# MaxChen228/pingpong-selfplay-ai

Hardware: AMD Instinct MI355X
Metric: env-steps/sec (whole node) at 65536 arenas, 1/2/4/8 GPUs; CPU-ref baseline (higher is better)
Workload: dtype f64 env state / f32 QNet; 1 GPU; configs[2]: 65536 arenas/GPU, full DQN train_iterative loop (act both players + env tick + PER push/sample + double-DQN update + Adam + target sync); arenas_per_gpu=65536, global_arenas=65536, pool=8, batch=256, updates_per_vector_step=1, memory_size=1000000, parallelism=dp1 (arena shards, 1 all-reduce/update)

## Files before the change

### pingpong-selfplay-ai_amd/csrc/pm_mfma.h

```cpp
#pragma once
#include "pm_dev.h"

namespace pm {

typedef float f32x16 __attribute__((ext_vector_type(16)));
typedef __attribute__((address_space(3))) void lds_void;

constexpr int PLAIN = 4936;
enum : int {
    F_W1 = 0,
    F_W2 = 512,
    F_B1 = 4608,
    F_B2 = 4672,
    F_H = 4736,
    F_BH = 4992,
    F_SIZE = 5008,
};
static_assert(PLAIN + F_SIZE == PM_QNET_NW, "effective weight block size");

__device__ __forceinline__ int rho(int r) { return (r & 3) + 8 * (r >> 2); }

__device__ __forceinline__ float relu(float x) { return __int_as_float(max(__float_as_int(x), 0)); }

__device__ __forceinline__ void write_feature_frags(const float* __restrict__ p, float* __restrict__ w) {
// ... 242 lines not shown
    for (int t = 0; t < 2; ++t)
#pragma unroll
        for (int r = 0; r < 16; ++r) c1[t][r] = relu(c1[t][r]);
    {
        const float4* b = reinterpret_cast<const float4*>(lw + F_B2 + (jt * 2 + h) * 16);
#pragma unroll
        for (int q4 = 0; q4 < 4; ++q4) {
            const float4 v = b[q4];
            c2[4 * q4 + 0] = v.x; c2[4 * q4 + 1] = v.y; c2[4 * q4 + 2] = v.z; c2[4 * q4 + 3] = v.w;
        }
    }
    const float4* w2 = reinterpret_cast<const float4*>(lw + F_W2) + lane + jt * 8 * 64;
    float4 wcur = w2[0];
#pragma unroll
    for (int g = 0; g < 8; ++g) {
        const int t = g >> 2, rq = g & 3;
        const float4 wnext = w2[((g + 1) & 7) * 64];
        c2 = __builtin_amdgcn_mfma_f32_32x32x2f32(wcur.x, c1[t][4 * rq + 0], c2, 0, 0, 0);
        c2 = __builtin_amdgcn_mfma_f32_32x32x2f32(wcur.y, c1[t][4 * rq + 1], c2, 0, 0, 0);
        c2 = __builtin_amdgcn_mfma_f32_32x32x2f32(wcur.z, c1[t][4 * rq + 2], c2, 0, 0, 0);
        c2 = __builtin_amdgcn_mfma_f32_32x32x2f32(wcur.w, c1[t][4 * rq + 3], c2, 0, 0, 0);
        wcur = wnext;
        __builtin_amdgcn_sched_barrier(0);
    }
}

__device__ __forceinline__ void heads_half(const float* hf, const f32x16& c2, int lane, int t, float (&acc)[4]) {
    const float4* hw = reinterpret_cast<const float4*>(hf + (lane >> 5) * 128) + t * 16;
#pragma unroll
    for (int r = 0; r < 16; ++r) {
        const float x = relu(c2[r]);
        const float4 w = hw[r];
        acc[0] = fmaf(w.x, x, acc[0]);
        acc[1] = fmaf(w.y, x, acc[1]);
        acc[2] = fmaf(w.z, x, acc[2]);
        acc[3] = fmaf(w.w, x, acc[3]);
    }
}

__device__ __forceinline__ void heads_finish(const float (&acc)[4], const float* hf, float (&q)[3]) {
    float v = acc[0], a0 = acc[1], a1 = acc[2], a2 = acc[3];
    v += __shfl_xor(v, 32);
    a0 += __shfl_xor(a0, 32);
    a1 += __shfl_xor(a1, 32);
    a2 += __shfl_xor(a2, 32);
    v += hf[256];
    a0 += hf[257];
    a1 += hf[258];
    a2 += hf[259];
    const float mean = ((a0 + a1) + a2) / 3.0f;
    q[0] = v + (a0 - mean);
    q[1] = v + (a1 - mean);
    q[2] = v + (a2 - mean);
}

__device__ __forceinline__ void tile_inputs(const float* __restrict__ o, int h, float (&xs)[4]) {
    xs[0] = h ? o[0] : 1.0f;
    xs[1] = o[1 + h];
    xs[2] = o[3 + h];
    xs[3] = o[5 + h];
}

struct TilePre {
    bool have;
    float xs[4];
};

__device__ __forceinline__ void run_tiles(const float* lw, const float* __restrict__ obs, const int* list, int count,
                                          const TileOut& out, const TilePre pre) {
    const int lane = threadIdx.x & 63, wave = threadIdx.x >> 6, nw = blockDim.x >> 6;
    const int h = lane >> 5, col = lane & 31;
    const int ntiles = (count + 31) >> 5;
    int tl = wave;
    if (tl >= ntiles) return;
    int arena = list[min(tl * 32 + col, count - 1)];
    float xs[4];
    if (pre.have) {
#pragma unroll
        for (int k = 0; k < 4; ++k) xs[k] = pre.xs[k];
    } else {
        tile_inputs(obs + (size_t)arena * 7, h, xs);
    }
    for (; tl < ntiles; tl += nw) {
        const int row = tl * 32 + col;
        const bool valid = row < count;
        const int tn = tl + nw;
        int arena_n = arena;
        float xn[4] = {xs[0], xs[1], xs[2], xs[3]};
        if (tn < ntiles) {
            arena_n = list[min(tn * 32 + col, count - 1)];
            tile_inputs(obs + (size_t)arena_n * 7, h, xn);
        }
        f32x16 c2[2];
#ifdef PM_DIAG
        if (tl == wave) {
            __builtin_amdgcn_s_waitcnt(0);
            PM_BLK(5);
        }
#endif
        tile_hidden(lw, xs, lane, c2);
#ifdef PM_DIAG
        if (tl == wave) PM_BLK(6);
#endif
        float q[3];
        tile_heads(lw + F_H, c2, lane, q);
#ifdef PM_DIAG
// ... 164 lines not shown
```

### pingpong-selfplay-ai_amd/csrc/pm_rollout.hip

```cpp
#include "pm_host.h"
#include "pm_mfma.h"
#include "pm_per.h"

using namespace pm;

namespace {

constexpr int kRollBlock = 256;
constexpr int kHeadsBlock = 256;
static_assert(PM_ROLL_HEADS == 264, "heads workspace stride: 256 fragment floats + 4 biases + 4 pad");

__global__ __launch_bounds__(kHeadsBlock) void k_rollout_heads(const float* __restrict__ paramsB, uint64_t seed_net,
                                                               uint64_t counter0, float* __restrict__ ws) {
    __shared__ float noise[132];
    __shared__ float heads[260];
    gen_noise(seed_net, TAG_NOISE_ACT, counter0 + blockIdx.x, noise, threadIdx.x, blockDim.x);
    __syncthreads();
    fold_heads_from(paramsB + PM_QNET_HEAD_OFF, nullptr, noise, PM_FOLD_TRAIN_FRESH, heads, nullptr, threadIdx.x,
                    blockDim.x);
    __syncthreads();
    float* hf = ws + (size_t)blockIdx.x * PM_ROLL_HEADS;
    heads_to_frags(heads, hf);
    if (threadIdx.x < 4) hf[260 + threadIdx.x] = 0.f;
}
// ... 176 lines not shown
            if (lane < 32)
#pragma unroll
                for (int k = 0; k < 7; ++k) { sm.ob[0][col][k] = oA[k]; sm.ob[1][col][k] = nB2[k]; }
        } else if (st + 1 < steps) {
            roll_draws(p, sm, i, ctr + 1, (st + 1) & 1, eps, seed_env, wv, lane);
        }
        __syncthreads();
    }
    if (wv == 3 && lane < 32 && valid) {
        store_arena(s, i, a);
        float oA[7], oB[7];
        observe(a, oA, oB);
        store_row7(obsA + (size_t)i * 7, oA);
        store_row7(obsB + (size_t)i * 7, oB);
        rp.ep_reward[i] = er;
    }
    if (!stats) return;
    const bool mine = wv == 3 && lane < 32 && valid;
    long long v[6] = {mine ? fin : 0, mine ? winB : 0, mine ? ptA : 0, mine ? ptB : 0, mine ? winE : 0,
                      mine ? rsum : 0};
#pragma unroll
    for (int k = 0; k < 6; ++k) v[k] = wave_sum(v[k]);
    long long mv = v[0];
#pragma unroll
    for (int k = 1; k < 6; ++k) mv = lane == k ? v[k] : mv;
    if (wv == 3 && lane < 6) atomicAdd(reinterpret_cast<unsigned long long*>(stats + lane), (unsigned long long)mv);
}

__global__ __launch_bounds__(kRollBlock) __attribute__((amdgpu_waves_per_eu(3, 3))) void k_rollout_push(
    const pm_env_params p, const pm_env_state s, const float* __restrict__ wA, const float* __restrict__ wB,
    const float* __restrict__ ws, double eps, uint64_t seed_env, uint64_t counter0, int steps,
    float* __restrict__ obsA, float* __restrict__ obsB, long long* __restrict__ stats, int n, const RollPush rp) {
    rollout_push_body(p, s, wA, wB, ws, eps, seed_env, counter0, steps, obsA, obsB, stats, n, rp);
}

constexpr int kR16Block = 512;

#ifdef PM_DIAG
static __device__ unsigned long long pm_diag_roll[2][8];
#define ROLL_T(k)                                                                 \
    do {                                                                          \
        if (diag) {                                                               \
            const unsigned long long now_ = __builtin_amdgcn_s_memtime();         \
            dacc[(k)] += now_ - dprev;                                            \
            dprev = now_;                                                         \
        }                                                                         \
    } while (0)
#else
#define ROLL_T(k) \
    do {          \
    } while (0)
#endif

__device__ __forceinline__ int l2_pos(int u) {
    const int t = u >> 5, v = u & 31, b = (v >> 2) & 1, r = (v & 3) + 4 * (v >> 3);
    return 2 * (16 * t + r) + b;
}
__device__ __forceinline__ int l2_unit(int q) {
    const int i = q >> 1, b = q & 1;
    return 32 * (i >> 4) + rho(i & 15) + 4 * b;
}
__device__ __forceinline__ int head_pos(int u) {
    const int t = u >> 5, v = u & 31;
    return 16 * t + (v & 3) + 4 * (v >> 3);
}

typedef float f32x4v16 __attribute__((ext_vector_type(4)));

struct Roll16Shared {
    __attribute__((aligned(16))) float img2[2][4][4][64][4];
    __attribute__((aligned(16))) float img1[2][4][64][2];
    __attribute__((aligned(16))) float b2v[2][4][4][4];
    __attribute__((aligned(16))) float hfA[264];
    __attribute__((aligned(16))) float hfB[2][320];
    __attribute__((aligned(16))) float h1s[2][4][4][16][4];
    __attribute__((aligned(16))) float c2s[2][2][8][16][4];
    float ob[2][16][8];
    ServeDraw sdraw[2][16];
    int epsa[2][16];
    __attribute__((aligned(16))) float opw[3][2][4][32];
};

__device__ __forceinline__ void roll16_opw(Roll16Shared& sm, int set, const float* hf) {
    const int lane = threadIdx.x & 63;
#pragma unroll
    for (int it = 0; it < 4; ++it) {
        const int idx = it * 64 + lane, h = idx >> 7, j = (idx >> 5) & 3, q = idx & 31;
        sm.opw[set][h][j][q] = hf[(h * 32 + q) * 4 + j];
    }
}

__device__ __forceinline__ float xor16_sum(float v) {
    const auto r = __builtin_amdgcn_permlane16_swap(__float_as_uint(v), __float_as_uint(v), false, false);
    return __uint_as_float(r[0]) + __uint_as_float(r[1]);
}
__device__ __forceinline__ void halves_bcast(int v, int& lo, int& hi) {
    const auto r = __builtin_amdgcn_permlane32_swap((unsigned)v, (unsigned)v, false, false);
    lo = (int)r[0];
    hi = (int)r[1];
}

__device__ __forceinline__ void roll16_serve(const pm_env_params& p, Roll16Shared& sm, int i, uint64_t ctr, int b,
                                             uint64_t seed, int g) {
    const U4 r = philox((uint32_t)i, g == 1 ? (TAG_SERVE_STEP | 0x100u) : TAG_SERVE_STEP, (uint32_t)ctr,
                        (uint32_t)(ctr >> 32), seed);
    const auto sx = __builtin_amdgcn_permlane16_swap(r.x, r.x, false, false);
    const auto sy = __builtin_amdgcn_permlane16_swap(r.y, r.y, false, false);
    const auto sz = __builtin_amdgcn_permlane16_swap(r.z, r.z, false, false);
    const auto sw = __builtin_amdgcn_permlane16_swap(r.w, r.w, false, false);
    const ServeDraw d = serve_from_blocks(p, r, U4{sx[1], sy[1], sz[1], sw[1]});
    if (g == 0) sm.sdraw[b][threadIdx.x & 15] = d;
}
__device__ __forceinline__ void roll16_eps(Roll16Shared& sm, int i, uint64_t ctr, int b, double eps, uint64_t seed,
                                           int g) {
    if (g == 0) {
        const U4 rr = philox64((uint32_t)i, TAG_ACT, ctr, seed);
        sm.epsa[b][threadIdx.x & 15] = u53(rr.x, rr.y) < eps ? (int)below(rr.z, 3u) : -1;
    }
}

__device__ __forceinline__ void rollout16_body(const pm_env_params& p, const pm_env_state& s, const float* __restrict__ wA,
                                               const float* __restrict__ wB, const float* __restrict__ ws, double eps,
                                               uint64_t seed_env, uint64_t counter0, int steps, float* __restrict__ obsA,
                                               float* __restrict__ obsB, long long* __restrict__ stats, int n) {
    __shared__ Roll16Shared sm;
    const int t = threadIdx.x, lane = t & 63, col = lane & 15, g = lane >> 4;
    const int wv = __builtin_amdgcn_readfirstlane(t >> 6);
    const int player = wv >> 2, rt = wv & 3;
    const int i = blockIdx.x * 16 + col;
    const bool valid = i < n;
    for (int k = t; k < 2 * 4 * 4 * 64 * 4; k += kR16Block) {
        const int pp = k >> 12, r2 = (k >> 10) & 3, s4 = (k >> 8) & 3, ln = (k >> 2) & 63, e = k & 3;
        const float* w = pp ? wB : wA;
        (&sm.img2[0][0][0][0][0])[k] = w[W2 + (16 * r2 + (ln & 15)) * 64 + l2_unit(4 * (4 * s4 + e) + (ln >> 4))];
    }
    for (int k = t; k < 2 * 4 * 64 * 2; k += kR16Block) {
        const int pp = k >> 9, r2 = (k >> 7) & 3, ln = (k >> 1) & 63, sx = k & 1;
        const float* w = pp ? wB : wA;
        const int row = 16 * r2 + (ln & 15), kk = 4 * sx + (ln >> 4);
        (&sm.img1[0][0][0][0])[k] = kk == 0 ? w[B1 + row] : w[W1 + row * 7 + kk - 1];
    }
    if (t < 128) {
        const int pp = t >> 6, r2 = (t >> 4) & 3, gg = (t >> 2) & 3, r = t & 3;
        (&sm.b2v[0][0][0][0])[t] = (pp ? wB : wA)[B2 + 16 * r2 + 4 * gg + r];
    }
    if (t < 260) sm.hfA[t] = t < 256 ? wA[PLAIN + F_H + t] : wA[PLAIN + F_BH + t - 256];
    if (wv == 7) fetch_heads(ws, 0, sm.hfB[0], lane);
    if (wv == 1) roll16_serve(p, sm, i, counter0, 0, seed_env, g);
    if (wv == 2) roll16_eps(sm, i, counter0, 0, eps, seed_env, g);
    Arena a{};
    int fin = 0, winB = 0, ptA = 0, ptB = 0;
    if (wv == 0) {
        a = load_arena(s, valid ? i : n - 1);
        float oA[7], oB[7];
        observe(a, oA, oB);
        if (g < 2)
#pragma unroll
            for (int k = 0; k < 7; ++k) sm.ob[g][col][k] = g ? oB[k] : oA[k];
    }
    asm volatile("s_waitcnt vmcnt(0)" ::: "memory");
    if (wv == 7) roll16_opw(sm, 1, sm.hfB[0]);
    if (wv == 6) roll16_opw(sm, 0, wA + PLAIN + F_H);
    __syncthreads();
    const float4* im2 = reinterpret_cast<const float4*>(sm.img2[player][rt][0][lane]);
    float4 w2r[4];
    const float2 w1r = *reinterpret_cast<const float2*>(sm.img1[player][rt][lane]);
#pragma unroll
    for (int s4 = 0; s4 < 4; ++s4) {
        const float4 w = im2[s4 * 64];
        w2r[s4] = w;
    }
    const float4 b2r = *reinterpret_cast<const float4*>(sm.b2v[player][rt][g]);
#ifdef PM_DIAG
    const bool diag = blockIdx.x == 0 && wv < 2;
    unsigned long long dacc[8] = {0, 0, 0, 0, 0, 0, 0, 0}, dprev = __builtin_amdgcn_s_memtime();
#endif
    for (int st = 0; st < steps; ++st) {
        const uint64_t ctr = counter0 + (uint64_t)st;
        if (wv == 7 && st + 1 < steps) fetch_heads_async(ws, st + 1, sm.hfB[(st + 1) & 1], lane);
        float hw4[32];
        if (wv == 0) {
            const float* src = sm.opw[(lane >> 5) ? 1 + (st & 1) : 0][(lane >> 4) & 1][lane & 3];
#pragma unroll
            for (int k = 0; k < 8; ++k) {
                const float4 w = *reinterpret_cast<const float4*>(src + 4 * k);
                hw4[4 * k] = w.x; hw4[4 * k + 1] = w.y; hw4[4 * k + 2] = w.z; hw4[4 * k + 3] = w.w;
            }
        }
        {
            const float* o = sm.ob[player][col];
            const float o0 = o[g == 0 ? 0 : g - 1];
            const float x0 = g == 0 ? 1.0f : o0, x1 = o[3 + g];
            const f32x4v16 zero = {0.f, 0.f, 0.f, 0.f};
            f32x4v16 c1 = __builtin_amdgcn_mfma_f32_16x16x4f32(w1r.x, x0, zero, 0, 0, 0);
            c1 = __builtin_amdgcn_mfma_f32_16x16x4f32(w1r.y, x1, c1, 0, 0, 0);
#pragma unroll
            for (int r = 0; r < 4; ++r) {
                const int q = l2_pos(16 * rt + 4 * g + r), sq = q >> 2;
                sm.h1s[player][q & 3][sq >> 2][col][sq & 3] = relu(c1[r]);
            }
        }
        ROLL_T(0);
        __syncthreads();
        ROLL_T(1);
        float bs[16];
        {
#pragma unroll
            for (int k = 0; k < 4; ++k) {
                const float4 v = *reinterpret_cast<const float4*>(sm.h1s[player][g][k][col]);
                bs[4 * k] = v.x; bs[4 * k + 1] = v.y; bs[4 * k + 2] = v.z; bs[4 * k + 3] = v.w;
            }
        }
        f32x4v16 c2 = {b2r.x, b2r.y, b2r.z, b2r.w};

#pragma unroll
// ... 13 lines not shown
        if (wv == 7) asm volatile("s_waitcnt vmcnt(0)" ::: "memory");
        ROLL_T(2);
        __syncthreads();
        ROLL_T(3);
        if (wv == 0) {
            const int hp = lane >> 5, hh = (lane >> 4) & 1;
            const float* hf = hp ? sm.hfB[st & 1] : sm.hfA;
            float xb[32];
#pragma unroll
            for (int k = 0; k < 8; ++k) {
                const float4 x = *reinterpret_cast<const float4*>(sm.c2s[hp][hh][k][col]);
                xb[4 * k] = x.x; xb[4 * k + 1] = x.y; xb[4 * k + 2] = x.z; xb[4 * k + 3] = x.w;
            }
            const int ea = sm.epsa[st & 1][col];
            ServeDraw sd = sm.sdraw[st & 1][col];
            f32x4v16 acc = {0.f, 0.f, 0.f, 0.f};
#pragma unroll
            for (int q = 0; q < 32; ++q) acc = __builtin_amdgcn_mfma_f32_4x4x1f32(hw4[q], xb[q], acc, 0, 0, 0);
            __builtin_amdgcn_sched_group_barrier(0x100, 9, 0);
            __builtin_amdgcn_sched_group_barrier(0x008, 32, 0);
            float v = xor16_sum(acc[0]), a0 = xor16_sum(acc[1]), a1 = xor16_sum(acc[2]), a2 = xor16_sum(acc[3]);
            v += hf[256];
            a0 += hf[257];
            a1 += hf[258];
            a2 += hf[259];
            const float mean = ((a0 + a1) + a2) / 3.0f;
            const float qv[3] = {v + (a0 - mean), v + (a1 - mean), v + (a2 - mean)};
            int act = argmax3(qv);
            if (hp) act = ea >= 0 ? ea : act;
            int aA, aB;
            halves_bcast(act, aA, aB);
            ROLL_T(4);
            float rA, rB;
            const int d = tick(p, a, aA, aB, rA, rB);
            ptA += rA > 0.f ? 1 : 0;
            ptB += rB > 0.f ? 1 : 0;
            if (d) {
                fin += 1;
                winB += rB > 0.f ? 1 : 0;
                serve_finish(sd);
                serve(a, sd.vx, sd.vy, sd.spin);
            }
            float oA[7], oB[7];
            observe(a, oA, oB);
            if (g < 2)
#pragma unroll
                for (int k = 0; k < 7; ++k) sm.ob[g][col][k] = g ? oB[k] : oA[k];
            ROLL_T(5);
        } else if (wv == 1 && st + 1 < steps) {
            roll16_serve(p, sm, i, ctr + 1, (st + 1) & 1, seed_env, g);
        } else if (wv == 2 && st + 1 < steps) {
            roll16_eps(sm, i, ctr + 1, (st + 1) & 1, eps, seed_env, g);
        } else if (wv == 7 && st + 1 < steps) {
            roll16_opw(sm, 1 + ((st + 1) & 1), sm.hfB[(st + 1) & 1]);
        }
        __syncthreads();
        ROLL_T(6);
    }
#ifdef PM_DIAG
    if (diag && lane == 0)
#pragma unroll
        for (int k = 0; k < 8; ++k) pm_diag_roll[wv][k] = k < 7 ? dacc[k] : (unsigned long long)steps;
#endif
    if (wv == 0 && g == 0 && valid) {
        store_arena(s, i, a);
        float oA[7], oB[7];
        observe(a, oA, oB);
        store_row7(obsA + (size_t)i * 7, oA);
        store_row7(obsB + (size_t)i * 7, oB);
    }
    if (!stats || wv != 0) return;
    const bool mine = g == 0 && valid;
    long long v[4] = {mine ? fin : 0, mine ? winB : 0, mine ? ptA : 0, mine ? ptB : 0};
#pragma unroll
    for (int k = 0; k < 4; ++k) v[k] = wave_sum(v[k]);
    long long mv = v[0];
#pragma unroll
    for (int k = 1; k < 4; ++k) mv = lane == k ? v[k] : mv;
    if (lane < 4) atomicAdd(reinterpret_cast<unsigned long long*>(stats + lane), (unsigned long long)mv);
}

__global__ __launch_bounds__(kR16Block) void k_rollout16(const pm_env_params p, const pm_env_state s,
                                                         const float* __restrict__ wA, const float* __restrict__ wB,
                                                         const float* __restrict__ ws, double eps, uint64_t seed_env,
                                                         uint64_t counter0, int steps, float* __restrict__ obsA,
                                                         float* __restrict__ obsB, long long* __restrict__ stats,
                                                         int n) {
    rollout16_body(p, s, wA, wB, ws, eps, seed_env, counter0, steps, obsA, obsB, stats, n);
}

}

static int rollout_launch(const pm_env_params* p, const pm_env_state* s, const float* wA, const float* wB,
                          const float* paramsB, float epsilon, uint64_t seed_env, uint64_t seed_net, uint64_t counter0,
                          int32_t steps, float* heads_ws, float* obsA, float* obsB, const RollPush* rp, void* per_work,
                          int64_t* stats, int32_t n, void* stream) {
    const char* name = rp ? "pm_rollout_push" : "pm_rollout";
    PM_REQUIRE(n >= 0 && steps >= 0, PM_E_SIZE, "%s: n=%d steps=%d", name, n, steps);
    if (n == 0 || steps == 0) return PM_OK;
    PM_REQUIRE(p && s && s->x && s->y && s->vx && s->vy && s->spin && s->top && s->bot && s->scoreA && s->scoreB &&
                   s->bounces && wA && wB && paramsB && heads_ws && obsA && obsB,
               PM_E_ARG, "%s: null buffer", name);
    PM_REQUIRE((((uintptr_t)wA) | ((uintptr_t)wB) | ((uintptr_t)heads_ws)) % 16 == 0, PM_E_ARG,
               "%s: wA, wB and heads_ws must be 16-byte aligned", name);
    PM_REQUIRE(p->speed_scale_every > 0, PM_E_ARG, "%s: speed_scale_every must be > 0", name);
    hipStream_t st = pm_stream(stream);
    hipLaunchKernelGGL(k_rollout_heads, dim3(steps), dim3(kHeadsBlock), 0, st, paramsB, seed_net, counter0, heads_ws);
// ... 48 lines not shown
```

### pingpong-selfplay-ai_amd/csrc/pm_selfplay.hip

```cpp
#include <algorithm>
#include <cmath>

#include "pm_host.h"
#include "pm_mfma.h"
#include "pm_per.h"

using namespace pm;

#ifdef PM_DIAG
static __device__ unsigned long long pm_diag_env[8][1024];
static __device__ unsigned long long pm_diag_side[4][1024];
#define PM_SIDE(k, sb, v)                                                        \
    do {                                                                         \
        if (threadIdx.x == 0 && (sb) < 1024) pm_diag_side[(k)][(sb)] = (v);      \
    } while (0)
#define PM_STAMP_MAX_NB(slot)                                                                              \
    do {                                                                                                   \
        if (threadIdx.x == 0) atomicMax(&pm_diag_buf[(slot)], (unsigned long long)__builtin_amdgcn_s_memrealtime()); \
    } while (0)
#define PM_ENV_STAMP(k, blk)                                                                   \
    do {                                                                                       \
        asm volatile("" ::: "memory");                                                         \
        if (threadIdx.x == 0 && (blk) < 1024) pm_diag_env[(k)][(blk)] = __builtin_amdgcn_s_memrealtime(); \
    } while (0)
// ... 176 lines not shown
    rb[0] = tr[7];
    rb[1] = tr[15];
    tile_hidden(lw, xs, lane, c2);
    tile_heads(hf0, c2, lane, qb);
    tile_heads(hf1, c2, lane, qt);
}

template <bool WT = false>
__device__ __forceinline__ void store_hfeat(float* hfeat, int j, bool nxt, int lane, const f32x16 (&c2)[2],
                                            const float (&qb)[3], const float (&qt)[3], const float (&rb)[2]) {
    float* row = hfeat + (size_t)j * 80;
    const int h = lane >> 5;
    if (!nxt) {
#pragma unroll
        for (int t = 0; t < 2; ++t)
#pragma unroll
            for (int q = 0; q < 16; ++q) st_out<WT>(&row[32 * t + rho(q) + 4 * h], relu(c2[t][q]));
    }
    if (h == 0) {
        if (!nxt) {
            st_out<WT>(&row[64], qb[0]); st_out<WT>(&row[65], qb[1]); st_out<WT>(&row[66], qb[2]);
            st_out<WT>(&row[67], rb[0]);
            st_out<WT>(&row[71], rb[1]);
        } else {
            st_out<WT>(&row[68], qb[0]); st_out<WT>(&row[69], qb[1]); st_out<WT>(&row[70], qb[2]);
            st_out<WT>(&row[72], qt[0]); st_out<WT>(&row[73], qt[1]); st_out<WT>(&row[74], qt[2]);
        }
    }
}

__device__ __forceinline__ void env_fwd_block(const pm_selfplay& sp, int f, bool pending = true) {
    __shared__ __attribute__((aligned(16))) float lw[kLwFloats];
    __shared__ __attribute__((aligned(16))) float hf[2][264];
    if (!learner_active(sp)) return;
    stage_frags_lds(sp.w_B, lw, f * 5);
    for (int k = threadIdx.x; k < 2 * 264; k += blockDim.x) hf[k / 264][k % 264] = sp.learn_heads[k];
    __syncthreads();
    const int lane = threadIdx.x & 63, B = sp.batch;
    const int r0 = f * 128 + (int)(threadIdx.x >> 6) * 32;
    if (r0 >= 2 * B) return;
    const int r = min(r0 + (lane & 31), 2 * B - 1);
    const bool nxt = r >= B;
    const int j = nxt ? r - B : r;
    const int64_t id = sp.idx[j];
    const pm_ctrl* c = sp.ctrl;
    const bool mine = r0 + (lane & 31) < 2 * B && !(pending && push_of(sp, c->pos, c->size, c->max_prio).covers(id));
    f32x16 c2[2];
    float qb[3], qt[3];
    float rb[2];
    batch_row_fwd(sp, lw, hf[0], hf[1], id, nxt, lane, c2, qb, qt, rb);
    if (mine) store_hfeat(sp.hfeat, j, nxt, lane, c2, qb, qt, rb);
}

struct SampleFwd32Smem {
    PerSampleSmem per;
    float lw[kLwFloats];
    float hf[pad256(2 * 264)];
    int64_t sidx[PER_BS / 2];
    float part[2][64][8];
};
__device__ __forceinline__ void sample_fwd_block32(const pm_selfplay& sp, int b, SampleFwd32Smem& sm) {
    constexpr int NS = PER_BS / 2;
    const pm_ctrl* c = sp.ctrl;
    const int64_t csize = c->size, cpos = c->pos, cframe = c->frame_idx;
    const float cmaxp = c->max_prio;
    const int64_t s = csize + sp.n;
    const int64_t size = s < sp.cap ? s : sp.cap;
    const int64_t frame = cframe + 1;
    const bool active = size >= sp.batch;
    const PushRange pr = push_of(sp, cpos, csize, cmaxp);
    const double beta = beta_of(sp, frame);
    const uint64_t key = sp.seed_env;
    int wj = -1;
    double wpa = 0.0, wtot = 1.0;
    per_sample_block<true>(
        active, size, per_tree(sp.per_work, sp.cap), pr, beta, b * NS, min(sp.batch, b * NS + NS), sm.per,
        [&](int j) {
            const U4 r = philox64((uint32_t)j, TAG_PER, (uint64_t)frame, key);
            return u53(r.x, r.y);
        },
        [&](int j, int64_t idx, double pa, double total) {
            sp.idx[j] = idx;
            sm.sidx[j - b * NS] = idx;
            wj = j;
            wpa = pa;
            wtot = total;
        },
        [&] {
            stage_frags_lds(sp.w_B, sm.lw, b * 5);
            copy_lds_f32x4<2 * 264>(sp.learn_heads, sm.hf);
        });
    if (!active) return;
    __syncthreads();
    PM_BLK(1);
    const int lane = threadIdx.x & 63, B = sp.batch;
    const int wv = __builtin_amdgcn_readfirstlane(threadIdx.x >> 6);
    const bool nxt = (wv >> 1) != 0;
    const int jt = wv & 1;
    const int j = b * NS + (lane & 31);
    const int64_t id = sm.sidx[min(j, B - 1) - b * NS];
    const bool mine = j < B && !pr.covers(id);
    const int h = lane >> 5;
    float xs[4];
    const float* tr = sp.trans + id * PM_TRANS_F;
    tile_inputs(tr + (nxt ? 8 : 0), h, xs);
    const float rb0 = tr[7], rb1 = tr[15];
    if (wj >= 0) sp.isw[wj] = per_is_weight(size, wpa, wtot, beta);
    f32x16 c2;
    hidden_half(sm.lw, xs, lane, jt, c2);
    const float* hf0 = sm.hf;
    const float* hf1 = sm.hf + 264;
    float ab[4] = {0.f, 0.f, 0.f, 0.f}, at[4] = {0.f, 0.f, 0.f, 0.f};
    float* row = sp.hfeat + (size_t)j * 80;
    if (jt == 0) {
        heads_half(hf0, c2, lane, 0, ab);
        if (nxt) heads_half(hf1, c2, lane, 0, at);
        *reinterpret_cast<float4*>(&sm.part[nxt][lane][0]) = make_float4(ab[0], ab[1], ab[2], ab[3]);
        if (nxt) *reinterpret_cast<float4*>(&sm.part[nxt][lane][4]) = make_float4(at[0], at[1], at[2], at[3]);
    }
    if (mine && !nxt) {
#pragma unroll
        for (int q = 0; q < 16; ++q) row[32 * jt + rho(q) + 4 * h] = relu(c2[q]);
    }
    __syncthreads();
    if (jt == 0) return;
    {
        const float4 pa = *reinterpret_cast<const float4*>(&sm.part[nxt][lane][0]);
        ab[0] = pa.x; ab[1] = pa.y; ab[2] = pa.z; ab[3] = pa.w;
    }
    heads_half(hf0, c2, lane, 1, ab);
    float qb[3], qt[3];
    heads_finish(ab, hf0, qb);
    if (nxt) {
        const float4 pt = *reinterpret_cast<const float4*>(&sm.part[nxt][lane][4]);
        at[0] = pt.x; at[1] = pt.y; at[2] = pt.z; at[3] = pt.w;
        heads_half(hf1, c2, lane, 1, at);
        heads_finish(at, hf1, qt);
    }
    if (mine && h == 0) {
        if (!nxt) {
            row[64] = qb[0]; row[65] = qb[1]; row[66] = qb[2];
            row[67] = rb0;
            row[71] = rb1;
        } else {
            row[68] = qb[0]; row[69] = qb[1]; row[70] = qb[2];
            row[72] = qt[0]; row[73] = qt[1]; row[74] = qt[2];
        }
    }
}

__device__ __forceinline__ void write_opp_lists(const pm_selfplay& sp, OppListSmem& sm, int blk, int i, bool valid,
                                                int net) {
    write_opp_lists(sp.n_pool + 1, sp.opp_list, sp.opp_cnt, sm, blk, i, valid, net);
}

struct EnvSmem {
    float lds[2][kBlock][7];
    long long red[kBlock / 64][6];
    OppListSmem ol;
};
struct ActEnvSmem {
    EnvSmem e;
    float lw[kLwFloats];
};

template <bool ACT>
__device__ __forceinline__ void env_block(const pm_selfplay& sp, int blk, EnvSmem& sm, float* lw) {
    const int i0 = blk * kBlock;
    const int i = i0 + threadIdx.x;
    const int lane = threadIdx.x & 63, wv = threadIdx.x >> 6;
    const bool valid = i < sp.n;
    const int ii = valid ? i : sp.n - 1;
    const pm_ctrl* c = sp.ctrl;
    if (blk == 0) PM_STAMP_ANY(72);
    PM_ENV_STAMP(0, blk);
    float xs[2][4];
    f32x16 fc2[2][2];
    const bool ahead = ACT && gb_current(sp);
    if (ahead) {
    } else if (ACT && sp.featB) {
        if (threadIdx.x < 65)
            reinterpret_cast<float4*>(lw + F_H)[threadIdx.x] =
                reinterpret_cast<const float4*>(sp.w_B + PLAIN + F_H)[threadIdx.x];
        const int tlast = feat_ntiles(sp.n) - 1;
#pragma unroll
        for (int k = 0; k < 2; ++k) feat_load(sp.featB, min(blk * 8 + 2 * wv + k, tlast), lane, fc2[k]);
    } else if (ACT) {
        stage_frags_lds(sp.w_B, lw, blk);
#pragma unroll
        for (int k = 0; k < 2; ++k) {
            const int row = min(i0 + 64 * wv + 32 * k + (lane & 31), sp.n - 1);
            tile_inputs(sp.obsB + (size_t)row * 7, lane >> 5, xs[k]);
        }
    }
    const uint32_t ns = (uint32_t)__builtin_nontemporal_load(&sp.st.serves[ii]);
    const int64_t pos = c->pos, size = c->size;
    const float cmaxp = c->max_prio;
    const uint64_t cstep = c->step;
    const double ceps = c->epsilon;
// ... 95 lines not shown
    if (valid) {
        int64_t slot = pos + i;
        if (slot >= sp.cap) slot -= sp.cap;
        float4* row = reinterpret_cast<float4*>(sp.trans + slot * PM_TRANS_F);
        st_f4<kEnvWTRows>(row + 0, make_float4(oB[0], oB[1], oB[2], oB[3]));
        st_f4<kEnvWTRows>(row + 1, make_float4(oB[4], oB[5], oB[6], rB));
        st_f4<kEnvWTRows>(row + 2, make_float4(nB[0], nB[1], nB[2], nB[3]));
        st_f4<kEnvWTRows>(row + 3, make_float4(nB[4], nB[5], nB[6], __int_as_float(aB | (d << 8))));
        sp.prios[slot] = maxp;
        leaf[slot] = pval;
        float ernew = er;
        if (d) {
            onew = onext;
            serve(a, svx, svy, sspn);
            sp.st.serves[i] = (int32_t)ns + 1;
            ernew = 0.f;
            observe(a, nA, nB);
        }
        store_arena<kEnvWTState>(sp.st, i, a);
        sp.opp[i] = onew;
        sp.aB[i] = (int8_t)aB;
        sp.ep_reward[i] = ernew;
    }
    PM_ENV_STAMP(3, blk);
#pragma unroll
    for (int k = 0; k < 7; ++k) { sm.lds[0][threadIdx.x][k] = nA[k]; sm.lds[1][threadIdx.x][k] = nB[k]; }
    __syncthreads();
    PM_ENV_STAMP(4, blk);
    if (threadIdx.x < 6) {
        long long t = 0;
        for (int w = 0; w < kBlock / 64; ++w) t += sm.red[w][threadIdx.x];
        sp.partials[(size_t)blk * 8 + threadIdx.x] = t;
    }
    write_opp_lists(sp, sm.ol, blk, i, valid, onew);
    PM_ENV_STAMP(5, blk);
    copy_rows7<kEnvWTObs>(sp.obsA, sm.lds[0], i0, sp.n);
    copy_rows7<kEnvWTObs>(sp.obsB, sm.lds[1], i0, sp.n);
    PM_ENV_STAMP_DRAIN(6, blk);
}

__global__ __launch_bounds__(kBlock) void k_env(const pm_selfplay sp) {
    const int blk = (int)blockIdx.x;
    const int nenv = (sp.n + kBlock - 1) / kBlock;
    if (blk >= nenv) {
        env_fwd_block(sp, blk - nenv);
        return;
    }
    __shared__ __attribute__((aligned(16))) EnvSmem sm;
    env_block<false>(sp, blk, sm, nullptr);
}

union ActEnvShared {
    ActEnvSmem ae;
    SampleFwd32Smem sf32;
};
__global__ __launch_bounds__(kBlock) void k_actenv(const pm_selfplay sp) {
    __shared__ __attribute__((aligned(16))) ActEnvShared sh;
    const int nsb = (sp.batch + 31) / 32;
    if ((int)blockIdx.x < nsb) {
        PM_BLK(0);
        sample_fwd_block32(sp, (int)blockIdx.x, sh.sf32);
        PM_BLK_END();
        return;
    }
    env_block<true>(sp, (int)blockIdx.x - nsb, sh.ae.e, sh.ae.lw);
}

__global__ __launch_bounds__(kBlock) void k_sp_init(const pm_selfplay sp) {
    __shared__ __attribute__((aligned(16))) float lds[kBlock][7];
    const int i0 = blockIdx.x * kBlock;
    const int i = i0 + threadIdx.x;
    float oA[7] = {0}, oB[7] = {0};
    int net = 0;
    if (i < sp.n) {
        const uint32_t ns = (uint32_t)sp.st.serves[i];
        const U4 q = philox((uint32_t)i, TAG_OPP, ns, 0u, sp.seed_env);
        net = (sp.n_pool > 0 && u53(q.x, q.y) < sp.pool_ratio) ? 1 + below(q.z, (uint32_t)sp.n_pool) : 0;
        sp.opp[i] = net;
        Arena a;
        double vx, vy, spn;
        philox_serve(sp.env, (uint32_t)i, ns, sp.seed_env, vx, vy, spn);
        serve(a, vx, vy, spn);
        store_arena(sp.st, i, a);
        sp.st.serves[i] = (int32_t)ns + 1;
        sp.ep_reward[i] = 0.f;
        observe(a, oA, oB);
    }
    {
        __shared__ OppListSmem ol;
        write_opp_lists(sp, ol, blockIdx.x, i, i < sp.n, net);
    }
    store_rows7(sp.obsA, lds, oA, i0, sp.n);
    store_rows7(sp.obsB, lds, oB, i0, sp.n);
}

struct __attribute__((aligned(16))) ApplySmem {
    float hp[pad256(PM_QNET_NHEAD)];
    float tmu[pad256(PM_QNET_NHEAD)];
    float m[pad256(PM_QNET_NHEAD)], v[pad256(PM_QNET_NHEAD)];
    float g[PM_QNET_NHEAD + 2];
    float ak[2];
    float nact[132], ntrain[132];
    float heads[3][260];
    double eps_next;
};

__device__ __forceinline__ void adam_consts(const pm_selfplay& sp, int64_t ts, ApplySmem& sm) {
    const double bc1 = 1.0 - pow(sp.beta1, (double)ts);
    const double bc2 = 1.0 - pow(sp.beta2, (double)ts);
    sm.ak[0] = (float)(sp.lr / bc1);
    sm.ak[1] = (float)sqrt(bc2);
}
__device__ __forceinline__ void adam_const_lane(const pm_selfplay& sp, int64_t ts, ApplySmem& sm, int which) {
    const double bc = 1.0 - pow(which ? sp.beta2 : sp.beta1, (double)ts);
// ... 1727 lines not shown
unsigned learn_blocks(const pm_selfplay* sp, bool with_act, const LearnGrid& lg) {
    unsigned blocks = 2u + (with_act ? (unsigned)lg.g.blocks() : 0u);
    if (with_act && sp->featB) blocks += (unsigned)((feat_ntiles(sp->n) + lg.ftiles - 1) / lg.ftiles);
    return blocks;
}

int act_ahead(const pm_selfplay* sp, int mode, bool with_act, const LearnGrid& lg) {
    if (!with_act || !sp->fuse_apply || mode != (PM_UPD_FIRST | PM_UPD_LAST) || !sp->featB || !sp->gB || !sp->gheads ||
        sp->frow || lg.ftiles > 2 * (kLearn / 64) || (int)learn_blocks(sp, with_act, lg) > device_cus())
        return 0;
    const char* e = getenv("PONGMI_ACT_AHEAD");
    if (e && *e && atoi(e) == 0) return 0;
    const char* f = getenv("PONGMI_AHEAD_FORCE_TIMEOUT");
    return 1 | ((f && *f && atoi(f) != 0) << 1);
}

int launch_learn(const pm_selfplay* sp, bool with_act, hipStream_t st, int mode = PM_UPD_FIRST | PM_UPD_LAST) {
    const LearnGrid lg = learn_grid(sp);
    const ActGrid& g = lg.g;
    const unsigned blocks = learn_blocks(sp, with_act, lg);
    const int tr = tree_refresh_block();
    const int ahead = act_ahead(sp, mode, with_act, lg);
    pm_launch(PM_TIMER_LEARN, (tr & 8) ? k_learn<true> : k_learn<false>, dim3(blocks), dim3(kLearn), st, *sp, g.chunk0,
              g.chunk1, mode, tr, lg.ftiles, side_sleep(ahead & 1), ahead);
    PM_LAUNCHED("k_learn");
    return PM_OK;
}
}

extern "C" int pm_selfplay_act(const pm_selfplay* sp, void* stream) {
    return pm_selfplay_act_part(sp, PM_ACT_ALL, stream);
}

extern "C" int pm_selfplay_act_part(const pm_selfplay* sp, int32_t part, void* stream) {
    int rc = check(sp);
    if (rc) return rc;
    PM_REQUIRE(part == PM_ACT_ALL || part == PM_ACT_B || part == PM_ACT_A, PM_E_ARG,
               "pm_selfplay_act_part: part=%d", part);
    return launch_act(sp, part, pm_stream(stream));
}

extern "C" int pm_selfplay_env(const pm_selfplay* sp, void* stream) {
    int rc = check(sp);
    if (rc) return rc;
    const unsigned nfwd = pm_blocks(2 * sp->batch, 128);
    hipLaunchKernelGGL(k_env, dim3(pm_blocks(sp->n, kBlock) + nfwd), dim3(kBlock), 0, pm_stream(stream), *sp);
    PM_LAUNCHED("k_env");
    return PM_OK;
}

extern "C" int pm_selfplay_actenv(const pm_selfplay* sp, void* stream) {
    int rc = check(sp);
    if (rc) return rc;
    const unsigned nsb = pm_blocks(sp->batch, 32);
    pm_launch(PM_TIMER_ACTENV, k_actenv, dim3(nsb + pm_blocks(sp->n, kBlock)), dim3(kBlock), pm_stream(stream), *sp);
    PM_LAUNCHED("k_actenv");
    return PM_OK;
}

extern "C" int pm_selfplay_rollout(const pm_selfplay* sp, void* stream) {
    int rc = pm_selfplay_act(sp, stream);
    return rc ? rc : pm_selfplay_env(sp, stream);
}

extern "C" int pm_selfplay_learn(const pm_selfplay* sp, void* stream) {
    int rc = check(sp);
    return rc ? rc : launch_learn(sp, false, pm_stream(stream));
}

extern "C" int pm_selfplay_learn_act(const pm_selfplay* sp, void* stream) {
    int rc = check(sp);
    return rc ? rc : launch_learn(sp, true, pm_stream(stream));
}

extern "C" int pm_selfplay_act_ahead(const pm_selfplay* sp, int32_t mode, int32_t with_act) {
    if (check(sp)) return 0;
    return act_ahead(sp, (int)mode, with_act != 0, learn_grid(sp)) & 1;
}

extern "C" int pm_selfplay_apply(const pm_selfplay* sp, void* stream) {
    return pm_selfplay_apply_ex(sp, PM_UPD_FIRST | PM_UPD_LAST, stream);
}

extern "C" int pm_selfplay_apply_ex(const pm_selfplay* sp, int32_t mode, void* stream) {
    int rc = check(sp);
    if (rc) return rc;
    PM_REQUIRE(mode >= 0 && mode <= (PM_UPD_FIRST | PM_UPD_LAST), PM_E_ARG, "pm_selfplay_apply_ex: mode=%d", mode);
    if (sp->fuse_apply) return PM_OK;
    hipLaunchKernelGGL(k_adam, dim3(1), dim3(kLearn), 0, pm_stream(stream), *sp, (int)mode);
    PM_LAUNCHED("k_adam");
    return PM_OK;
}

extern "C" int pm_selfplay_learn_ex(const pm_selfplay* sp, int32_t mode, int32_t with_act, void* stream) {
    int rc = check(sp);
    if (rc) return rc;
    PM_REQUIRE(mode >= 0 && mode <= (PM_UPD_FIRST | PM_UPD_LAST), PM_E_ARG, "pm_selfplay_learn_ex: mode=%d", mode);
    return launch_learn(sp, with_act != 0, pm_stream(stream), (int)mode);
}

extern "C" int pm_selfplay_resample(const pm_selfplay* sp, void* stream) {
    int rc = check(sp);
    if (rc) return rc;
    hipStream_t st = pm_stream(stream);
    hipLaunchKernelGGL(k_resample, dim3((sp->batch + PER_BS - 1) / PER_BS), dim3(256), 0, st, *sp);
    PM_LAUNCHED("k_resample");
    hipLaunchKernelGGL(k_batch_fwd, dim3(pm_blocks(2 * sp->batch, 128)), dim3(kBlock), 0, st, *sp);
// ... 71 lines not shown
```

Measured before the change: 2.112 billion env-steps/s.

## Rewrite PER sample forward as 8-sample MFMA 16x16x4 blocks with register weights

Replaces the 32-sample-per-block sample forward pass with blocks of 8 samples (cur and next states packed into 16 columns). The layers now run through mfma_f32_16x16x4f32 and the heads through mfma 4x4x1, with weights loaded straight into registers instead of being staged whole into LDS. This launches four times as many small sample blocks so the PER forward spreads across more CUs and overlaps with the env blocks in the fused actenv kernel. Shared helpers move into pm_mfma.h. The trade-off is more blocks each re-reading the weights, plus an extra barrier for the hidden-layer exchange.

Result: faster. 2.195 billion env-steps/s, median of 6 (+3.9%).

```diff
diff --git a/pingpong-selfplay-ai_amd/csrc/pm_mfma.h b/pingpong-selfplay-ai_amd/csrc/pm_mfma.h
--- a/pingpong-selfplay-ai_amd/csrc/pm_mfma.h
+++ b/pingpong-selfplay-ai_amd/csrc/pm_mfma.h
@@ -318,6 +318,36 @@
     q[0] = v + (a0 - mean);
     q[1] = v + (a1 - mean);
     q[2] = v + (a2 - mean);
+}
+
+__device__ __forceinline__ int l2_pos(int u) {
+    const int t = u >> 5, v = u & 31, b = (v >> 2) & 1, r = (v & 3) + 4 * (v >> 3);
+    return 2 * (16 * t + r) + b;
+}
+__device__ __forceinline__ int l2_unit(int q) {
+    const int i = q >> 1, b = q & 1;
+    return 32 * (i >> 4) + rho(i & 15) + 4 * b;
+}
+__device__ __forceinline__ int head_pos(int u) {
+    const int t = u >> 5, v = u & 31;
+    return 16 * t + (v & 3) + 4 * (v >> 3);
+}
+
+typedef float f32x4v16 __attribute__((ext_vector_type(4)));
+
+template <int NSET>
+__device__ __forceinline__ void heads_to_opw(float (&opw)[NSET][2][4][32], int set, const float* hf) {
+    const int lane = threadIdx.x & 63;
+#pragma unroll
+    for (int it = 0; it < 4; ++it) {
+        const int idx = it * 64 + lane, h = idx >> 7, j = (idx >> 5) & 3, q = idx & 31;
+        opw[set][h][j][q] = hf[(h * 32 + q) * 4 + j];
+    }
+}
+
+__device__ __forceinline__ float xor16_sum(float v) {
+    const auto r = __builtin_amdgcn_permlane16_swap(__float_as_uint(v), __float_as_uint(v), false, false);
+    return __uint_as_float(r[0]) + __uint_as_float(r[1]);
 }
 
 __device__ __forceinline__ void tile_inputs(const float* __restrict__ o, int h, float (&xs)[4]) {
diff --git a/pingpong-selfplay-ai_amd/csrc/pm_rollout.hip b/pingpong-selfplay-ai_amd/csrc/pm_rollout.hip
--- a/pingpong-selfplay-ai_amd/csrc/pm_rollout.hip
+++ b/pingpong-selfplay-ai_amd/csrc/pm_rollout.hip
@@ -252,21 +252,6 @@
     } while (0)
 #endif
 
-__device__ __forceinline__ int l2_pos(int u) {
-    const int t = u >> 5, v = u & 31, b = (v >> 2) & 1, r = (v & 3) + 4 * (v >> 3);
-    return 2 * (16 * t + r) + b;
-}
-__device__ __forceinline__ int l2_unit(int q) {
-    const int i = q >> 1, b = q & 1;
-    return 32 * (i >> 4) + rho(i & 15) + 4 * b;
-}
-__device__ __forceinline__ int head_pos(int u) {
-    const int t = u >> 5, v = u & 31;
-    return 16 * t + (v & 3) + 4 * (v >> 3);
-}
-
-typedef float f32x4v16 __attribute__((ext_vector_type(4)));
-
 struct Roll16Shared {
     __attribute__((aligned(16))) float img2[2][4][4][64][4];
     __attribute__((aligned(16))) float img1[2][4][64][2];
@@ -281,19 +266,6 @@
     __attribute__((aligned(16))) float opw[3][2][4][32];
 };
 
-__device__ __forceinline__ void roll16_opw(Roll16Shared& sm, int set, const float* hf) {
-    const int lane = threadIdx.x & 63;
-#pragma unroll
-    for (int it = 0; it < 4; ++it) {
-        const int idx = it * 64 + lane, h = idx >> 7, j = (idx >> 5) & 3, q = idx & 31;
-        sm.opw[set][h][j][q] = hf[(h * 32 + q) * 4 + j];
-    }
-}
-
-__device__ __forceinline__ float xor16_sum(float v) {
-    const auto r = __builtin_amdgcn_permlane16_swap(__float_as_uint(v), __float_as_uint(v), false, false);
-    return __uint_as_float(r[0]) + __uint_as_float(r[1]);
-}
 __device__ __forceinline__ void halves_bcast(int v, int& lo, int& hi) {
     const auto r = __builtin_amdgcn_permlane32_swap((unsigned)v, (unsigned)v, false, false);
     lo = (int)r[0];
@@ -359,8 +331,8 @@
             for (int k = 0; k < 7; ++k) sm.ob[g][col][k] = g ? oB[k] : oA[k];
     }
     asm volatile("s_waitcnt vmcnt(0)" ::: "memory");
-    if (wv == 7) roll16_opw(sm, 1, sm.hfB[0]);
-    if (wv == 6) roll16_opw(sm, 0, wA + PLAIN + F_H);
+    if (wv == 7) heads_to_opw(sm.opw, 1, sm.hfB[0]);
+    if (wv == 6) heads_to_opw(sm.opw, 0, wA + PLAIN + F_H);
     __syncthreads();
     const float4* im2 = reinterpret_cast<const float4*>(sm.img2[player][rt][0][lane]);
     float4 w2r[4];
@@ -480,7 +452,7 @@
         } else if (wv == 2 && st + 1 < steps) {
             roll16_eps(sm, i, ctr + 1, (st + 1) & 1, eps, seed_env, g);
         } else if (wv == 7 && st + 1 < steps) {
-            roll16_opw(sm, 1 + ((st + 1) & 1), sm.hfB[(st + 1) & 1]);
+            heads_to_opw(sm.opw, 1 + ((st + 1) & 1), sm.hfB[(st + 1) & 1]);
         }
         __syncthreads();
         ROLL_T(6);
diff --git a/pingpong-selfplay-ai_amd/csrc/pm_selfplay.hip b/pingpong-selfplay-ai_amd/csrc/pm_selfplay.hip
--- a/pingpong-selfplay-ai_amd/csrc/pm_selfplay.hip
+++ b/pingpong-selfplay-ai_amd/csrc/pm_selfplay.hip
@@ -252,15 +252,17 @@
     if (mine) store_hfeat(sp.hfeat, j, nxt, lane, c2, qb, qt, rb);
 }
 
-struct SampleFwd32Smem {
+constexpr int kSampBlock = 8;
+struct SampleFwd16Smem {
     PerSampleSmem per;
-    float lw[kLwFloats];
-    float hf[pad256(2 * 264)];
-    int64_t sidx[PER_BS / 2];
-    float part[2][64][8];
+    int64_t sidx[kSampBlock];
+    __attribute__((aligned(16))) float h1s[4][4][16][4];
+    __attribute__((aligned(16))) float c2s[2][8][16][4];
+    __attribute__((aligned(16))) float hf[pad256(2 * 264)];
+    __attribute__((aligned(16))) float opw[2][2][4][32];
 };
-__device__ __forceinline__ void sample_fwd_block32(const pm_selfplay& sp, int b, SampleFwd32Smem& sm) {
-    constexpr int NS = PER_BS / 2;
+__device__ __forceinline__ void sample_fwd_block16(const pm_selfplay& sp, int b, SampleFwd16Smem& sm) {
+    constexpr int NS = kSampBlock;
     const pm_ctrl* c = sp.ctrl;
     const int64_t csize = c->size, cpos = c->pos, cframe = c->frame_idx;
     const float cmaxp = c->max_prio;
@@ -271,8 +273,13 @@
     const PushRange pr = push_of(sp, cpos, csize, cmaxp);
     const double beta = beta_of(sp, frame);
     const uint64_t key = sp.seed_env;
+    const int lane = threadIdx.x & 63, col = lane & 15, g = lane >> 4;
+    const int rt = __builtin_amdgcn_readfirstlane(threadIdx.x >> 6);
     int wj = -1;
     double wpa = 0.0, wtot = 1.0;
+    float4 f1 = make_float4(0.f, 0.f, 0.f, 0.f), f2[8], b2r = f1;
+#pragma unroll
+    for (int m = 0; m < 8; ++m) f2[m] = f1;
     per_sample_block<true>(
         active, size, per_tree(sp.per_work, sp.cap), pr, beta, b * NS, min(sp.batch, b * NS + NS), sm.per,
         [&](int j) {
@@ -287,64 +294,108 @@
             wtot = total;
         },
         [&] {
-            stage_frags_lds(sp.w_B, sm.lw, b * 5);
+            const float* w = sp.w_B;
+            const int jt = rt >> 1, fl = 32 * (g & 1) + 16 * (rt & 1) + col;
+            f1 = reinterpret_cast<const float4*>(w + PLAIN + F_W1)[jt * 64 + fl];
+            const float4* q2 = reinterpret_cast<const float4*>(w + PLAIN + F_W2) + jt * 8 * 64 + fl;
+#pragma unroll
+            for (int m = 0; m < 8; ++m) f2[m] = q2[m * 64];
+            b2r = *reinterpret_cast<const float4*>(w + B2 + 16 * rt + 4 * g);
             copy_lds_f32x4<2 * 264>(sp.learn_heads, sm.hf);
         });
     if (!active) return;
     __syncthreads();
     PM_BLK(1);
-    const int lane = threadIdx.x & 63, B = sp.batch;
-    const int wv = __builtin_amdgcn_readfirstlane(threadIdx.x >> 6);
-    const bool nxt = (wv >> 1) != 0;
-    const int jt = wv & 1;
-    const int j = b * NS + (lane & 31);
+    const int B = sp.batch;
+    const bool nxt = col >= NS;
+    const int j = b * NS + (col & (NS - 1));
     const int64_t id = sm.sidx[min(j, B - 1) - b * NS];
     const bool mine = j < B && !pr.covers(id);
-    const int h = lane >> 5;
-    float xs[4];
     const float* tr = sp.trans + id * PM_TRANS_F;
-    tile_inputs(tr + (nxt ? 8 : 0), h, xs);
+    const float* o = tr + (nxt ? 8 : 0);
+    const float o0 = o[g == 0 ? 0 : g - 1];
+    const float x1 = o[3 + g];
     const float rb0 = tr[7], rb1 = tr[15];
-    if (wj >= 0) sp.isw[wj] = per_is_weight(size, wpa, wtot, beta);
-    f32x16 c2;
-    hidden_half(sm.lw, xs, lane, jt, c2);
-    const float* hf0 = sm.hf;
-    const float* hf1 = sm.hf + 264;
-    float ab[4] = {0.f, 0.f, 0.f, 0.f}, at[4] = {0.f, 0.f, 0.f, 0.f};
+    if (rt >= 2) heads_to_opw(sm.opw, rt - 2, sm.hf + (rt - 2) * 264);
+    float wisw = 0.f;
+    if (wj >= 0) wisw = per_is_weight(size, wpa, wtot, beta);
+    const bool odd = (g >> 1) != 0;
+    const float w1r[2] = {odd ? f1.y : f1.x, odd ? f1.w : f1.z};
+    float w2r[16];
+#pragma unroll
+    for (int m = 0; m < 8; ++m) {
+        w2r[2 * m] = odd ? f2[m].y : f2[m].x;
+        w2r[2 * m + 1] = odd ? f2[m].w : f2[m].z;
+    }
+    {
+        const float x0 = g == 0 ? 1.0f : o0;
+        const f32x4v16 zero = {0.f, 0.f, 0.f, 0.f};
+        f32x4v16 c1 = __builtin_amdgcn_mfma_f32_16x16x4f32(w1r[0], x0, zero, 0, 0, 0);
+        c1 = __builtin_amdgcn_mfma_f32_16x16x4f32(w1r[1], x1, c1, 0, 0, 0);
+#pragma unroll
+        for (int r = 0; r < 4; ++r) {
+            const int q = l2_pos(16 * rt + 4 * g + r), sq = q >> 2;
+            sm.h1s[q & 3][sq >> 2][col][sq & 3] = relu(c1[r]);
+        }
+    }
+    __syncthreads();
+    float hw4[32];
+    {
+        const float* src = sm.opw[lane >> 5][(lane >> 4) & 1][lane & 3];
+#pragma unroll
+        for (int k = 0; k < 8; ++k) {
+            const float4 w = *reinterpret_cast<const float4*>(src + 4 * k);
+            hw4[4 * k] = w.x; hw4[4 * k + 1] = w.y; hw4[4 * k + 2] = w.z; hw4[4 * k + 3] = w.w;
+        }
+    }
+    const float4 bhr = *reinterpret_cast<const float4*>(sm.hf + (lane >> 5) * 264 + 256);
+    float bs[16];
+#pragma unroll
+    for (int k = 0; k < 4; ++k) {
+        const float4 v = *reinterpret_cast<const float4*>(sm.h1s[g][k][col]);
+        bs[4 * k] = v.x; bs[4 * k + 1] = v.y; bs[4 * k + 2] = v.z; bs[4 * k + 3] = v.w;
+    }
+    f32x4v16 c2 = {b2r.x, b2r.y, b2r.z, b2r.w};
+#pragma unroll
+    for (int i = 0; i < 16; ++i) c2 = __builtin_amdgcn_mfma_f32_16x16x4f32(w2r[i], bs[i], c2, 0, 0, 0);
     float* row = sp.hfeat + (size_t)j * 80;
-    if (jt == 0) {
-        heads_half(hf0, c2, lane, 0, ab);
-        if (nxt) heads_half(hf1, c2, lane, 0, at);
-        *reinterpret_cast<float4*>(&sm.part[nxt][lane][0]) = make_float4(ab[0], ab[1], ab[2], ab[3]);
-        if (nxt) *reinterpret_cast<float4*>(&sm.part[nxt][lane][4]) = make_float4(at[0], at[1], at[2], at[3]);
-    }
-    if (mine && !nxt) {
-#pragma unroll
-        for (int q = 0; q < 16; ++q) row[32 * jt + rho(q) + 4 * h] = relu(c2[q]);
-    }
-    __syncthreads();
-    if (jt == 0) return;
-    {
-        const float4 pa = *reinterpret_cast<const float4*>(&sm.part[nxt][lane][0]);
-        ab[0] = pa.x; ab[1] = pa.y; ab[2] = pa.z; ab[3] = pa.w;
-    }
-    heads_half(hf0, c2, lane, 1, ab);
-    float qb[3], qt[3];
-    heads_finish(ab, hf0, qb);
-    if (nxt) {
-        const float4 pt = *reinterpret_cast<const float4*>(&sm.part[nxt][lane][4]);
-        at[0] = pt.x; at[1] = pt.y; at[2] = pt.z; at[3] = pt.w;
-        heads_half(hf1, c2, lane, 1, at);
-        heads_finish(at, hf1, qt);
-    }
-    if (mine && h == 0) {
-        if (!nxt) {
-            row[64] = qb[0]; row[65] = qb[1]; row[66] = qb[2];
-            row[67] = rb0;
-            row[71] = rb1;
-        } else {
-            row[68] = qb[0]; row[69] = qb[1]; row[70] = qb[2];
-            row[72] = qt[0]; row[73] = qt[1]; row[74] = qt[2];
+#pragma unroll
+    for (int r = 0; r < 4; ++r) {
+        const int u = 16 * rt + 4 * g + r, q = head_pos(u);
+        c2[r] = relu(c2[r]);
+        sm.c2s[(u >> 2) & 1][q >> 2][col][q & 3] = c2[r];
+    }
+    if (mine && !nxt) *reinterpret_cast<float4*>(row + 16 * rt + 4 * g) = make_float4(c2[0], c2[1], c2[2], c2[3]);
+    __syncthreads();
+    if (rt != 0) return;
+    if (wj >= 0) sp.isw[wj] = wisw;
+    const int set = lane >> 5, hh = (lane >> 4) & 1;
+    float xb[32];
+#pragma unroll
+    for (int k = 0; k < 8; ++k) {
+        const float4 x = *reinterpret_cast<const float4*>(sm.c2s[hh][k][col]);
+        xb[4 * k] = x.x; xb[4 * k + 1] = x.y; xb[4 * k + 2] = x.z; xb[4 * k + 3] = x.w;
+    }
+    f32x4v16 acc = {0.f, 0.f, 0.f, 0.f};
+#pragma unroll
+    for (int q = 0; q < 32; ++q) acc = __builtin_amdgcn_mfma_f32_4x4x1f32(hw4[q], xb[q], acc, 0, 0, 0);
+    float v = xor16_sum(acc[0]), a0 = xor16_sum(acc[1]), a1 = xor16_sum(acc[2]), a2 = xor16_sum(acc[3]);
+    v += bhr.x;
+    a0 += bhr.y;
+    a1 += bhr.z;
+    a2 += bhr.w;
+    const float mean = ((a0 + a1) + a2) / 3.0f;
+    const float q0 = v + (a0 - mean), q1 = v + (a1 - mean), q2 = v + (a2 - mean);
+    if (mine && hh == 0) {
+        if (set == 0) {
+            float* qd = row + (nxt ? 68 : 64);
+            qd[0] = q0; qd[1] = q1; qd[2] = q2;
+            if (!nxt) {
+                row[67] = rb0;
+                row[71] = rb1;
+            }
+        } else if (nxt) {
+            row[72] = q0; row[73] = q1; row[74] = q2;
         }
     }
 }
@@ -546,14 +597,14 @@
 
 union ActEnvShared {
     ActEnvSmem ae;
-    SampleFwd32Smem sf32;
+    SampleFwd16Smem sf16;
 };
 __global__ __launch_bounds__(kBlock) void k_actenv(const pm_selfplay sp) {
     __shared__ __attribute__((aligned(16))) ActEnvShared sh;
-    const int nsb = (sp.batch + 31) / 32;
+    const int nsb = (sp.batch + kSampBlock - 1) / kSampBlock;
     if ((int)blockIdx.x < nsb) {
         PM_BLK(0);
-        sample_fwd_block32(sp, (int)blockIdx.x, sh.sf32);
+        sample_fwd_block16(sp, (int)blockIdx.x, sh.sf16);
         PM_BLK_END();
         return;
     }
@@ -2387,7 +2438,7 @@
 extern "C" int pm_selfplay_actenv(const pm_selfplay* sp, void* stream) {
     int rc = check(sp);
     if (rc) return rc;
-    const unsigned nsb = pm_blocks(sp->batch, 32);
+    const unsigned nsb = pm_blocks(sp->batch, kSampBlock);
     pm_launch(PM_TIMER_ACTENV, k_actenv, dim3(nsb + pm_blocks(sp->n, kBlock)), dim3(kBlock), pm_stream(stream), *sp);
     PM_LAUNCHED("k_actenv");
     return PM_OK;
```
